# lemma-osu/sknnr

Hardware: AMD Instinct MI355X
Metric: Mqueries/sec + achieved HBM GB/s, 10M×50k×32 k=5, 1/2/4/8 MI355X (higher is better)
Workload: dtype f16 split MFMA (hi.hi swept, lo.hi + hi.lo corrections; f32 accumulate) pre-filter + f64 exact re-score

## Files before the change

include/sknnr_hip.h:

```cpp
#ifndef SKNNR_HIP_H
#define SKNNR_HIP_H

#include <stdint.h>

#ifdef __cplusplus
extern "C" {
#endif
#pragma GCC visibility push(default)

#define SKNNR_ABI_VERSION 5

typedef enum sknnr_status {
    SKNNR_OK = 0,
    SKNNR_ERR_INVALID = -1,
    SKNNR_ERR_K_TOO_LARGE = -2,
    SKNNR_ERR_NO_TARGETS = -3,
    SKNNR_ERR_UNSUPPORTED = -4,
    SKNNR_ERR_HIP = -5,
    SKNNR_ERR_NO_DEVICE = -6,
    SKNNR_ERR_NONFINITE = -7
} sknnr_status;

typedef enum sknnr_memspace {
    SKNNR_MEM_HOST = 0,
// ... 124 lines not shown
int sknnr_crosswalk(const int64_t* table, int64_t n_table, const int64_t* idx, int64_t n,
                    int64_t* out, int32_t device, int32_t mem, void* stream);


int sknnr_debug_coarse_matrix(sknnr_index* index, const double* q, int64_t nq, float* out,
                              double* out_qnorm, double* out_scale, double* out_eps);

int sknnr_debug_last_prefilter(const sknnr_index* index, int64_t out[8]);

int sknnr_debug_last_finalize(const sknnr_index* index, int64_t out[4]);

int sknnr_debug_last_hamming(const sknnr_index* index, int64_t out[8]);

int sknnr_debug_last_scan(const sknnr_index* index, int64_t out[8]);

int sknnr_debug_hamming_candidates(const sknnr_index* index, int32_t* cnt, int32_t* ids, int64_t n);

int sknnr_debug_last_prep(const sknnr_index* index, int64_t out[8]);

int sknnr_debug_query_prep(const sknnr_index* index, int64_t n, void* qimg, double* qnc, double* xt, uint8_t* cell,
                           int32_t* perm, double* qnc_pos);

int sknnr_debug_image_constants(const sknnr_index* index, double* mu, double* s, int32_t* cell_depth, float* axes,
                                float* centre, float* thr);

#pragma GCC visibility pop
#ifdef __cplusplus
}
#endif
#endif
// ... 1 lines not shown
```

sknnr_amd/_build.py:

```python

from __future__ import annotations

import hashlib
import os
import shutil
import subprocess
import sys
from concurrent.futures import ThreadPoolExecutor

CSRC = os.path.join(os.path.dirname(os.path.abspath(__file__)), "csrc")
LIB_NAME = "libsknnr_hip.so"
LIB_PATH = os.path.join(CSRC, LIB_NAME)
OBJ_DIR = os.path.join(CSRC, "_obj")
UNITS = [
    ("host", "sknnr_hip.hip", []),
    ("k_exact", "k_exact.hip", []),
    ("k_hamming", "k_hamming.hip", []),
    ("k_forest", "k_forest.hip", []),
    ("k_coarse1", "k_coarse1.hip", []),
    ("k_coarse2_a", "k_coarse2.hip", ["-DSKNNR_C2_PART=0"]),
    ("k_coarse2_b", "k_coarse2.hip", ["-DSKNNR_C2_PART=1"]),
]
SOURCES = sorted({u[1] for u in UNITS})
HEADERS = ["launch.hip.h", "coarse.hip.h", "coarse2.hip.h", "bucket.hip.h", "hamming.hip.h", "exact.hip.h", "forest.hip.h",
           "../../include/sknnr_hip.h"]

HIPCC_FLAGS = [
    "--offload-arch=gfx950",
    "-O3",
    "-std=c++17",
    "-fPIC",
    "-ffp-contract=off",
    "-fvisibility=hidden",
    "-Wall",
    "-Wno-unused-function",
]


def hipcc_path() -> str:
# ... 71 lines not shown
```

sknnr_amd/_native.py:

```python

from __future__ import annotations

import ctypes
import os
from ctypes import POINTER, byref, c_char_p, c_double, c_float, c_int32, c_int64, c_void_p

import numpy as np

from . import _build

MEM_HOST = 0
MEM_DEVICE = 1
FORMULA_EXPANDED = 0
FORMULA_DIRECT = 1
FORMULA_HAMMING = 2
WEIGHTS_UNIFORM = 0
WEIGHTS_DISTANCE = 1
WEIGHTS_EXPLICIT = 2
WEIGHTS_F32_TARGETS = 0x100
WEIGHTS_F32_WEIGHTS = 0x200

ERR_INVALID = -1
ERR_K_TOO_LARGE = -2
ERR_NO_TARGETS = -3
# ... 37 lines not shown
    "sknnr_predict",
    "sknnr_predict_from_neighbors",
    "sknnr_hamming_distances",
    "sknnr_shard_candidates",
    "sknnr_merge_shards",
    "sknnr_stream_begin",
    "sknnr_stream_push",
    "sknnr_stream_flush",
    "sknnr_stream_end",
    "sknnr_crosswalk",
    "sknnr_debug_coarse_matrix",
    "sknnr_debug_last_prefilter",
    "sknnr_debug_last_finalize",
    "sknnr_debug_last_hamming",
    "sknnr_debug_last_scan",
    "sknnr_debug_hamming_candidates",
    "sknnr_debug_last_prep",
    "sknnr_debug_query_prep",
    "sknnr_debug_image_constants",
)


class QueryOpts(ctypes.Structure):
    _fields_ = [
        ("n_neighbors", c_int32),
        ("exclude_self", c_int32),
        ("deterministic", c_int32),
        ("decimals", c_int32),
        ("formula", c_int32),
        ("apply_affine", c_int32),
# ... 84 lines not shown
    lib.sknnr_predict.argtypes = [vp, vp, c_int64, POINTER(QueryOpts), vp, vp, vp, c_int32, vp]
    lib.sknnr_predict_from_neighbors.argtypes = [vp, vp, vp, vp, c_int64, c_int32, c_int32, vp,
                                                 c_int32, vp]
    lib.sknnr_hamming_distances.argtypes = [vp, vp, c_int64, vp, c_int64, vp, c_int32, vp]
    lib.sknnr_shard_candidates.argtypes = [vp, vp, c_int64, POINTER(QueryOpts), c_int64, vp, vp, c_int32, vp]
    lib.sknnr_merge_shards.argtypes = [vp, vp, c_int64, POINTER(QueryOpts), c_int32, vp, vp, vp, vp, c_int32, vp]
    lib.sknnr_crosswalk.argtypes = [vp, c_int64, vp, c_int64, vp, c_int32, c_int32, vp]
    lib.sknnr_debug_coarse_matrix.argtypes = [vp, vp, c_int64, vp, vp, POINTER(c_double),
                                              POINTER(c_double)]
    lib.sknnr_debug_last_prefilter.argtypes = [vp, POINTER(c_int64)]
    if hasattr(lib, "sknnr_debug_last_finalize"):
        lib.sknnr_debug_last_finalize.argtypes = [vp, POINTER(c_int64)]
    lib.sknnr_debug_last_hamming.argtypes = [vp, POINTER(c_int64)]
    if hasattr(lib, "sknnr_debug_last_scan"):
        lib.sknnr_debug_last_scan.argtypes = [vp, POINTER(c_int64)]
    lib.sknnr_debug_hamming_candidates.argtypes = [vp, vp, vp, c_int64]
    if hasattr(lib, "sknnr_debug_last_prep"):
        lib.sknnr_debug_last_prep.argtypes = [vp, POINTER(c_int64)]
        lib.sknnr_debug_query_prep.argtypes = [vp, c_int64, vp, vp, vp, vp, vp, vp]
        lib.sknnr_debug_image_constants.argtypes = [vp, vp, POINTER(c_double), POINTER(c_int32), vp, vp, vp]
    _lib = lib
    return lib


def check(code: int) -> None:
    if code != 0:
        raise HipBackendError(code, load().sknnr_last_error().decode("utf-8", "replace"))


def device_count() -> int:
# ... 81 lines not shown

    def forest_apply_host(self, q, query_dtype=0):
        q = _c_rows(q, QueryOpts(query_dtype=int(query_dtype)))
        out = np.empty((q.shape[0], self.d), dtype=np.float64)
        check(load().sknnr_forest_apply(self.handle, _host_ptr(q), q.shape[0], int(query_dtype), MEM_HOST,
                                        _host_ptr(out)))
        return out

    def forest_apply_device(self, q_ptr, nq, query_dtype, out_ptr):
        check(load().sknnr_forest_apply(self.handle, c_void_p(q_ptr or None), nq, int(query_dtype), MEM_DEVICE,
                                        c_void_p(out_ptr or None)))

    def stats(self) -> dict:
        st = Stats()
        check(load().sknnr_get_stats(self.handle, byref(st)))
        return st.as_dict()

    def reset_stats(self):
        check(load().sknnr_reset_stats(self.handle))

    @staticmethod
    def make_opts(k, exclude_self=False, deterministic=True, decimals=10, formula=FORMULA_EXPANDED,
                  apply_affine=False, weight_mode=WEIGHTS_UNIFORM, row_offset=0,
                  check_finite=False, query_dtype=0) -> QueryOpts:
        return QueryOpts(int(k), int(bool(exclude_self)), int(bool(deterministic)), int(decimals),
                         int(formula), int(bool(apply_affine)), int(weight_mode), int(bool(check_finite)),
                         int(query_dtype), 0, int(row_offset))

    def check_finite(self, stream=0) -> None:
        check(load().sknnr_check_finite(self.handle, c_void_p(stream or None)))

# ... 118 lines not shown
        return dict(zip(self.FINALIZE_FIELDS, (int(v) for v in out)))

    HAMMING_FIELDS = ("ran", "kk", "compacts", "seed_rows", "band", "tree_pairs", "chunks", "handed_to_scan")

    def debug_last_hamming(self) -> dict:
        out = (c_int64 * 8)()
        check(load().sknnr_debug_last_hamming(self.handle, out))
        return dict(zip(self.HAMMING_FIELDS, (int(v) for v in out)))

    SCAN_FIELDS = ("formula_plus_1", "chunked", "kk", "workgroups", "lds_bytes", "rows", "slices", "replayed_rows")

    def debug_last_scan(self) -> dict:
        out = (c_int64 * 8)()
        check(load().sknnr_debug_last_scan(self.handle, out))
        return dict(zip(self.SCAN_FIELDS, (int(v) for v in out)))

    def debug_hamming_candidates(self, n: int):
        cnt = np.empty(n, dtype=np.int32)
        ids = np.empty((n, 192), dtype=np.int32)
        check(load().sknnr_debug_hamming_candidates(self.handle, _host_ptr(cnt), _host_ptr(ids), int(n)))
        return cnt, ids

    PREP_FIELDS = ("kernel", "rows_per_block", "x_dtype", "nq", "nq_pad", "xt_written", "cells_by", "affine_bits")

    def debug_last_prep(self) -> dict:
        out = (c_int64 * 8)()
        check(load().sknnr_debug_last_prep(self.handle, out))
        return dict(zip(self.PREP_FIELDS, (int(v) for v in out)))

    def debug_query_prep(self, n: int, want=("qimg", "qnc", "xt", "cell", "perm", "qnc_pos")) -> dict:
# ... 124 lines not shown
```

sknnr_amd/csrc/exact.hip.h:

```cpp
#pragma once
#include <type_traits>
#include <hip/hip_runtime.h>
#include <float.h>
#include <math.h>
#include <stdint.h>

#include "bucket.hip.h"
#include "coarse.hip.h"

namespace sknnr {

enum : int { kDtypeF64 = 0, kDtypeF32 = 1, kDtypeI16 = 2, kDtypeU16 = 3, kDtypeU8 = 4, kDtypeI32 = 5, kDtypeCount = 6 };
__host__ __device__ constexpr int dtype_bytes(int dt) {
    return dt == kDtypeF64 ? 8 : (dt == kDtypeF32 || dt == kDtypeI32 ? 4 : (dt == kDtypeU8 ? 1 : 2));
}
__device__ __forceinline__ double load_as_f64(const void* __restrict__ x, int dt, long i) {
    switch (dt) {
        case kDtypeF32: return (double)((const float*)x)[i];
        case kDtypeI16: return (double)((const short*)x)[i];
        case kDtypeU16: return (double)((const unsigned short*)x)[i];
        case kDtypeU8: return (double)((const unsigned char*)x)[i];
        case kDtypeI32: return (double)((const int*)x)[i];
        default: return ((const double*)x)[i];
    }
// ... 356 lines not shown
    double s2;
    double inv_s;
    double eps_c;
    double ymax;
    double noise_a;
    double mu2;
    int* fail_list;
    int fail_base;
    int* fail_count;
    const int* qperm;
    long pos0;
    const unsigned long long* rec;
    const float* rec_bound;
    const double* qnc_pos;
    int* trunc_count;
};

constexpr int kDppQuadXor[4] = {0xE4, 0xB1, 0x4E, 0x1B};
constexpr int kDppRowHalfMirror = 0x141;
__device__ __forceinline__ int half_mirror8(int v) { return __builtin_amdgcn_update_dpp(0, v, kDppRowHalfMirror, 0xf, 0xf, false); }
template <int N>
__device__ __forceinline__ int peer8_i(int v, int mirror) {
    static_assert(N >= 1 && N < 8, "a peer of an 8-lane group");
    if constexpr (N < 4) {
        return __builtin_amdgcn_update_dpp(0, v, kDppQuadXor[N], 0xf, 0xf, false);
    } else if constexpr (N < 7) {
        return __builtin_amdgcn_update_dpp(0, mirror, kDppQuadXor[7 - N], 0xf, 0xf, false);
    } else {
        return mirror;
    }
}
// ... 202 lines not shown
    const double tau = group_min<LPQ>(rank >= s.kk - 1 ? d2 : INFINITY, c);
    const double bound = (qn + t_min - eps) * a.inv_s2 - noise;
    bool certified = (n_usable >= s.kk) && (tau < INFINITY) && (bound > tau);
    bool truncated = false;
    if constexpr (RECORD) {
        truncated = group_any<LPQ>(c == LPQ - 1 && need, (int)(threadIdx.x & 63) & ~(LPQ - 1));
        if (truncated) certified = false;
    }
    {
        const int gbase = (int)(threadIdx.x & 63) & ~(LPQ - 1);
        const double by_rank = scatter_d<LPQ>(d2, gbase + rank);
        const double next = __shfl_down(by_rank, 1, LPQ);
        const bool has_next = c + 1 < LPQ;
        const bool tied_here = has_next && by_rank == next && by_rank < INFINITY &&
                               (s.deterministic ? c == s.kk - 1 : c < s.kk);
        if (!s.raw && group_any<LPQ>(tied_here, gbase)) certified = false;
    }

    int sel = rank;
    const long self_id = s.row_offset + q;
    if (s.exclude_self) {
        const bool is_self = usable && (long)id == self_id && rank < s.kk;
        int drop = group_min_i<LPQ>(is_self ? rank : 0x7fffffff, c);
        if (drop == 0x7fffffff) drop = 0;
        sel = rank == drop ? -1 : (rank > drop ? rank - 1 : rank);
    }
    const bool chosen = usable && sel >= 0 && sel < s.k;
    const double dist = s.raw ? d2 : sqrt(d2 > 0.0 ? d2 : 0.0);

    int pos = sel;
    if (s.deterministic) {
// ... 13 lines not shown
            const PeersL<LPQ> k1_of(k1);
            const PeersI<LPQ> tag_of(tagged);
            for_each_peer<LPQ>([&](auto n) {
                const double k0j = k0_of.template get<n.value>();
                const long k1j = k1_of.template get<n.value>();
                const int tj = tag_of.template get<n.value>();
                const int ij = tj & 0x7fffffff;
                const bool less = (k0j < k0) || (k0j == k0 && (k1j < k1 || (k1j == k1 && ij < key_id)));
                pos += (tj < 0) && less;
            });
        }
    }
    if (live && chosen) {
        if (s.out_dist) s.out_dist[q * s.k + pos] = dist;
        s.out_idx[q * s.k + pos] = id + s.id_offset;
    }
    if (live && c == 0 && !certified) {
        const int slot = atomicAdd(a.fail_count, 1);
        a.fail_list[slot] = a.fail_base + (int)q;
        if (RECORD && truncated) atomicAdd(a.trunc_count, 1);
    }
}

#ifdef SKNNR_KERNELS_EXACT
__global__ void __launch_bounds__(256) finalize_record_kernel(FinalizeArgs a) {
    constexpr int LPQ = kRecordLen;
    const SelectArgs& s = a.s;
    const long gt = (long)blockIdx.x * 256 + threadIdx.x;
    long q = gt / LPQ;
    const int c = (int)(gt % LPQ);
    const bool live = q < s.nq;
    if (!live) q = s.nq - 1;
    const long q_list = a.qperm ? a.pos0 + q : q;
    const unsigned long long e = a.rec[q_list * LPQ + c];
    const float t_min = a.rec_bound[q_list];
// ... 684 lines not shown
```

sknnr_amd/csrc/k_exact.hip:

```cpp
#define SKNNR_KERNELS_EXACT 1
#include <cstdint>
#include <cstdlib>

#include "launch.hip.h"

namespace sknnr {
namespace {
__global__ void add_counter_kernel(const int* __restrict__ cnt, long long* __restrict__ total) { *total += *cnt; }

template <int BT>
hipError_t prep_lds_bt(const PrepArgs& a, hipStream_t st) {
    const size_t sh = (size_t)BT * (a.d_in | 1) * 8;
    hipError_t e = hipFuncSetAttribute((const void*)prep_queries_kernel<BT>, hipFuncAttributeMaxDynamicSharedMemorySize, (int)sh);
    if (e != hipSuccess) return e;
    prep_queries_kernel<BT><<<dim3((unsigned)(a.nq_pad / BT)), dim3(BT), sh, st>>>(a);
    return hipGetLastError();
}

template <int FORMULA>
hipError_t exact_scan_f(bool chunked, const ScanArgs& a, long blocks, size_t sh, hipStream_t st) {
    auto kern = chunked ? exact_scan_kernel<FORMULA, true> : exact_scan_kernel<FORMULA, false>;
    hipError_t e = hipFuncSetAttribute((const void*)kern, hipFuncAttributeMaxDynamicSharedMemorySize, (int)sh);
    if (e != hipSuccess) return e;
    kern<<<dim3((unsigned)blocks), dim3(kScanWaves * 64), sh, st>>>(a);
// ... 109 lines not shown
    return hipGetLastError();
}

hipError_t crosswalk(const long* table, const long* idx, long n, long* out, hipStream_t st) {
    const long want = (n + 255) / 256;
    const unsigned blocks = (unsigned)(want < 1 ? 1 : (want > 256L * 16 ? 256L * 16 : want));
    crosswalk_kernel<<<dim3(blocks), dim3(256), 0, st>>>(table, idx, n, out);
    return hipGetLastError();
}

hipError_t add_counter(const int* cnt, long long* total, hipStream_t st) {
    add_counter_kernel<<<dim3(1), dim3(1), 0, st>>>(cnt, total);
    return hipGetLastError();
}

}
}
```

sknnr_amd/csrc/launch.hip.h:

```cpp
#pragma once
#include <hip/hip_runtime.h>

#include "bucket.hip.h"
#include "coarse2.hip.h"
#include "exact.hip.h"
#include "forest.hip.h"
#include "hamming.hip.h"

namespace sknnr {
namespace launch {

hipError_t row_norms(const double* x, long n, int d, double* out, hipStream_t st);
hipError_t prep_direct(const PrepArgs& a, hipStream_t st);
hipError_t prep_lds(int rows_per_block, const PrepArgs& a, hipStream_t st);
hipError_t check_finite(const double* x, long n_el, int* status, hipStream_t st);
hipError_t cell_assign(const CellArgs& a, hipStream_t st);
hipError_t cell_count(const CellArgs& a, hipStream_t st);
hipError_t cell_scatter(const CellArgs& a, hipStream_t st);
hipError_t finalize(const FinalizeArgs& f, long n, hipStream_t st);
int finalize_lanes(const FinalizeArgs& f);
hipError_t exact_scan(int formula, bool chunked, const ScanArgs& a, long blocks, size_t lds_bytes, hipStream_t st);
hipError_t scan_merge(int formula, const ScanArgs& a, long blocks, size_t lds_bytes, int grid_wg_of_scan, int forced_slices,
                      hipStream_t st);
hipError_t pack_shards(const double* val, const long* idx, long nq, int n_shards, int kk, double* slice_v, int* slice_i,
                       hipStream_t st);
hipError_t predict(const PredictArgs& a, hipStream_t st);
hipError_t crosswalk(const long* table, const long* idx, long n, long* out, hipStream_t st);
hipError_t add_counter(const int* cnt, long long* total, hipStream_t st);

hipError_t hamming_pack(const double* xq, long nq, long nq_pad, int t, int tp, uint32_t* qimg, int* q_bad, hipStream_t st);
hipError_t hamming_rows(const double* x, long n, int t, int tpr, uint32_t* rows, hipStream_t st);
hipError_t hamming_coarse(const HammingArgs& a, hipStream_t st);
hipError_t hamming_rescore(const HammingRescoreArgs& a, hipStream_t st);
hipError_t hamming_distance_rows(const HammingRowsArgs& a, hipStream_t st);

hipError_t forest_apply(const ForestArgs& a, hipStream_t st);

struct Coarse1Launch {
    const char* rimg;
    int n_stages;
    const uint4* qimg;
    const double* qnc;
    float skip_scale;
// ... 33 lines not shown
```

sknnr_amd/csrc/sknnr_hip.hip:

```cpp
#include "../../include/sknnr_hip.h"

#include <hip/hip_runtime.h>
#include <sys/mman.h>

#include <algorithm>
#include <chrono>
#include <cmath>
#include <cstdarg>
#include <cstdio>
#include <cstdlib>
#include <condition_variable>
#include <cstring>
#include <deque>
#include <functional>
#include <future>
#include <limits>
#include <memory>
#include <mutex>
#include <new>
#include <string>
#include <thread>
#include <vector>

#include "launch.hip.h"
// ... 190 lines not shown
    DevBuf<int> perm2;
    int cell_depth = 0;
    DevBuf<float> cell_axes, cell_centre, cell_thr;
    DevBuf<int> cell_stage;
    DevBuf<unsigned char> qcell;
    DevBuf<int> qperm, cell_hist;

    DevBuf<double> xt, qnc, xstage, dist_stage, pred_stage;
    DevBuf<uint4> qimg;
    DevBuf<float> cand_val;
    DevBuf<int> cand_idx, fail_list, fail_count, fail_list2, slice_i;
    DevBuf<unsigned long long> rec;
    DevBuf<float> rec_bound;
    DevBuf<double> qnc_pos;
    DevBuf<double> slice_v;
    DevBuf<int> status;
    DevBuf<long long> fail_total;
    DevBuf<long> idx_stage;

    struct HostSlot {
        double* pin_x = nullptr;  size_t pin_x_n = 0;
        double* pin_d = nullptr;  size_t pin_d_n = 0;
        long* pin_i = nullptr;    size_t pin_i_n = 0;
        double* pin_p = nullptr;  size_t pin_p_n = 0;
        DevBuf<double> dev_x, dev_d, dev_p;
        DevBuf<long> dev_i;
        hipEvent_t ev_h2d = nullptr, ev_done = nullptr, ev_d2h = nullptr;
    } slot[kHostSlots];
    hipStream_t st_h2d = nullptr, st_run = nullptr, st_d2h = nullptr;
    std::unique_ptr<HostWorker> w_in, w_out;
// ... 34 lines not shown
                        &dist_stage, &pred_stage, &f_ids})
            b->release();
        f_nodes.release(); f_off.release(); f_depth.release();
        rimg.release();
        perm.release();
        perm2.release();
        cell_axes.release(); cell_centre.release(); cell_thr.release(); cell_stage.release();
        qcell.release(); qperm.release(); cell_hist.release();
        h_rimg.release(); h_wq.release(); h_qimg.release(); h_rrow.release(); h_bad.release(); h_cand_cnt.release(); h_cand_id.release();
        qimg.release();
        cand_val.release();
        cand_idx.release();
        rec.release(); rec_bound.release(); qnc_pos.release();
        fail_list.release();
        fail_count.release();
        fail_total.release();
        status.release();
        idx_stage.release();
        for (auto& sl : slot) {
            for (void* hp : {(void*)sl.pin_x, (void*)sl.pin_d, (void*)sl.pin_i, (void*)sl.pin_p})
                if (hp) (void)hipHostFree(hp);
            sl.dev_x.release(); sl.dev_d.release(); sl.dev_p.release(); sl.dev_i.release();
            for (hipEvent_t e : {sl.ev_h2d, sl.ev_done, sl.ev_d2h})
                if (e) (void)hipEventDestroy(e);
        }
        for (hipStream_t h : {st_h2d, st_run, st_d2h})
            if (h) (void)hipStreamDestroy(h);
        if (ev_ws) (void)hipEventDestroy(ev_ws);
        if (st_side) (void)hipStreamDestroy(st_side);
        for (hipEvent_t e : {ev_fork, ev_join})
// ... 507 lines not shown
        }
        {
            double m2 = 0.0;
            for (int c = 0; c < d; ++c) m2 += ix->mu[c] * ix->mu[c];
            ix->mu_norm = std::sqrt(m2) * (1.0 + 1e-12);
        }
        HIP_TRY(ix->rimg.ensure(img.size()));
        HIP_TRY(hipMemcpy(ix->rimg.p, img.data(), img.size(), hipMemcpyHostToDevice));
        HIP_TRY(ix->perm.ensure((size_t)n_ref));
        HIP_TRY(hipMemcpy(ix->perm.p, perm.data(), (size_t)n_ref * sizeof(int), hipMemcpyHostToDevice));
        HIP_TRY(ix->mu_dev.ensure(dp));
        HIP_TRY(hipMemcpy(ix->mu_dev.p, ix->mu.data(), dp * sizeof(double), hipMemcpyHostToDevice));
    }

    HIP_TRY(ix->fail_count.ensure(4));
    HIP_TRY(ix->fail_total.ensure(2));
    HIP_TRY(hipMemset(ix->fail_total.p, 0, 16));
    HIP_TRY(ix->status.ensure(4));
    HIP_TRY(hipMemset(ix->status.p, 0, 16));
    HIP_TRY(hipEventCreateWithFlags(&ix->ev_ws, hipEventDisableTiming));
    HIP_TRY(hipDeviceSynchronize());
    guard.p = nullptr;
    *out = ix;
    return SKNNR_OK;
}

extern "C" void sknnr_index_destroy(sknnr_index* ix) { delete ix; }

extern "C" int sknnr_index_set_affine(sknnr_index* ix, int32_t d_in, const double* center,
                                      const double* scale, const double* proj) {
// ... 546 lines not shown
        return fail(SKNNR_ERR_UNSUPPORTED, "n_neighbors = %d exceeds the HIP backend's limit of %d%s", o->n_neighbors,
                    kScanMaxKK - (o->exclude_self ? 1 : 0),
                    o->exclude_self ? " with X=None (the query rows' own rows are searched too)" : "");
    if (std::abs(o->decimals) > 300) return fail(SKNNR_ERR_INVALID, "decimals out of range");
    return SKNNR_OK;
}

int run_forest(sknnr_index* ix, const void* xdev, long nq, const sknnr_query_opts* o, double* d_dist, long* d_idx,
               hipStream_t st);
int run_device(sknnr_index* ix, const void* xdev, long nq, const sknnr_query_opts* o, double* d_dist,
               long* d_idx, hipStream_t st, int raw = 0, long id_offset = 0) {
    std::fill(std::begin(ix->last_prefilter), std::end(ix->last_prefilter), 0);
    std::fill(std::begin(ix->last_hamming), std::end(ix->last_hamming), 0);
    std::fill(std::begin(ix->last_finalize), std::end(ix->last_finalize), 0);
    std::fill(std::begin(ix->last_scan), std::end(ix->last_scan), 0);
    std::fill(std::begin(ix->last_prep), std::end(ix->last_prep), 0);
    ix->last_hamming_rows = 0;
    if (xdev && uses_forest(ix, o)) return run_forest(ix, xdev, nq, o, d_dist, d_idx, st);
    const int kk = o->n_neighbors + (o->exclude_self ? 1 : 0);
    const bool affine = o->apply_affine != 0 && xdev != nullptr;
    const bool self_rows = xdev == nullptr;
    const int x_dtype = self_rows ? kDtypeF64 : o->query_dtype;
    const bool to_xt = affine || x_dtype != kDtypeF64;
    static const bool scan_everything = std::getenv("SKNNR_EXACT_ONLY") != nullptr;
    const bool coarse = ix->ks > 0 && kk <= kCoarseMaxKK && o->formula != SKNNR_FORMULA_HAMMING && !scan_everything;
    const int d_x = affine ? ix->d_in : ix->d;
    if (nq > 0x7fffffffL) return fail(SKNNR_ERR_UNSUPPORTED, "more than 2^31 - 1 query rows in one call");
    if (affine && ix->ks == 0)
        return fail(SKNNR_ERR_UNSUPPORTED, "d = %d > 128 with an affine map is outside the HIP envelope", ix->d);
    if (ix->ws_busy) HIP_TRY(hipStreamWaitEvent(st, ix->ev_ws, 0));
// ... 15 lines not shown
        HIP_TRY(ix->qcell.ensure((size_t)cap_pad));
        HIP_TRY(ix->qperm.ensure((size_t)cap_pad));
    }
    const bool record = coarse && use_record(ix->ks, coarse_list_len(ix, kk), kk, use_coarse2(ix, coarse_list_len(ix, kk)), raw);
    if (record) {
        HIP_TRY(ix->rec.ensure((size_t)cap_pad * kRecordLen));
        HIP_TRY(ix->rec_bound.ensure((size_t)cap_pad));
        if (ix->cell_depth > 0) HIP_TRY(ix->qnc_pos.ensure((size_t)cap_pad));
    } else if (coarse) {
        HIP_TRY(ix->cand_val.ensure((size_t)cap_pad * 2 * coarse_list_len(ix, kk)));
        HIP_TRY(ix->cand_idx.ensure((size_t)cap_pad * 2 * coarse_list_len(ix, kk)));
    }
    if (coarse) {
        HIP_TRY(ix->fail_list.ensure(nq));
        HIP_TRY(hipMemsetAsync(ix->fail_count.p, 0, 16, st));
    }

    SelectArgs call{};
    call.xq = xq_call;
    call.ref = ix->ref64.p;
    call.rn = ix->rn64.p;
    call.nq = nq;
    call.d = ix->d;
    call.n_ref = (int)ix->n_ref;
    call.k = o->n_neighbors;
    call.kk = kk;
    call.exclude_self = o->exclude_self ? 1 : 0;
    call.deterministic = o->deterministic ? 1 : 0;
    call.formula = o->formula;
    call.pow10_is_divisor = o->decimals < 0;
// ... 106 lines not shown
            f.rec_bound = ix->rec_bound.p;
            f.qnc_pos = bucketed ? ix->qnc_pos.p : ix->qnc.p;
            f.trunc_count = ix->fail_count.p + 3;
        }
        f.m_list = coarse_list_len(ix, kk);
        f.rank_extra = coarse_rank_extra(f.m_list, kk);
        f.inv_s2 = 1.0 / (ix->s * ix->s);
        f.s2 = ix->s * ix->s;
        f.inv_s = 1.0 / ix->s;
        f.eps_c = (v2 ? eps_units2(ix->ks) : eps_units(ix->ks)) * std::ldexp(1.0, -24);
        f.ymax = ix->ymax;
        f.noise_a = (ix->d + 4) * std::ldexp(1.0, -53);
        f.mu2 = o->formula == SKNNR_FORMULA_EXPANDED ? 2.0 * ix->mu_norm : 0.0;
        f.fail_list = ix->fail_list.p;
        f.fail_count = ix->fail_count.p;
        f.fail_base = (int)c0;
        auto finalize_rows = [&](long r0, long rows, hipStream_t s_) {
            FinalizeArgs g = f;
            if (bucketed) {
                g.pos0 = r0;
                g.s.nq = rows;
                launch_finalize(g, rows, s_);
                return;
            }
            g.s.xq = f.s.xq + r0 * ix->d;
            g.s.nq = rows;
            g.s.row_offset = f.s.row_offset + r0;
            g.s.out_dist = f.s.out_dist ? f.s.out_dist + r0 * o->n_neighbors : nullptr;
            g.s.out_idx = f.s.out_idx + r0 * o->n_neighbors;
            if (record) {
// ... 10 lines not shown
        };
        ix->last_finalize[0] = launch::finalize_lanes(f);
        ix->last_finalize[1] = record ? 1 : 0;
        const long done = v2 ? std::min<long>(ix->bulk_rows_done, n) : 0;
        if (done > 0) {
            HIP_TRY(hipStreamWaitEvent(ix->st_side, ix->ev_fork, 0));
            finalize_rows(0, done, ix->st_side);
            HIP_TRY(hipGetLastError());
            HIP_TRY(hipEventRecord(ix->ev_join, ix->st_side));
            if (n > done) finalize_rows(done, n - done, st);
            HIP_TRY(hipGetLastError());
            HIP_TRY(hipStreamWaitEvent(st, ix->ev_join, 0));
        } else {
            finalize_rows(0, n, st);
            HIP_TRY(hipGetLastError());
        }
    }
    const bool ham_int = !coarse && o->formula == SKNNR_FORMULA_HAMMING && ix->h16_ok && kk <= kHamMaxKK;
    if (ham_int) {
        const long chunk_q = 1L << 18;
        const long cap_q = std::min(chunk_q, nq);
        const long cap_pad = (cap_q + 255) / 256 * 256;
        HIP_TRY(ix->h_qimg.ensure((size_t)ix->h_tp * cap_pad));
        HIP_TRY(ix->h_bad.ensure((size_t)cap_pad));
        HIP_TRY(ix->h_cand_cnt.ensure((size_t)cap_q));
        HIP_TRY(ix->h_cand_id.ensure((size_t)cap_q * kHamCand));
        HIP_TRY(ix->fail_list.ensure(nq));
        HIP_TRY(hipMemsetAsync(ix->fail_count.p, 0, 16, st));
        const int64_t rec[7] = {1, kk, ham_compacts(kk) ? 1 : 0, ham_seed_rows((int)ix->n_ref, kk), (int64_t)ix->d + 2,
                                ix->h_tp, (nq + chunk_q - 1) / chunk_q};
// ... 23 lines not shown
            hr.s.xq = xq_call + c0 * ix->d;
            hr.s.nq = n;
            hr.s.row_offset = o->row_offset + c0;
            hr.s.out_dist = d_dist ? d_dist + c0 * o->n_neighbors : nullptr;
            hr.s.out_idx = d_idx + c0 * o->n_neighbors;
            hr.cand_cnt = ix->h_cand_cnt.p;
            hr.cand_id = ix->h_cand_id.p;
            hr.fail_list = ix->fail_list.p;
            hr.fail_count = ix->fail_count.p;
            hr.fail_base = (int)c0;
            hr.rrow = ix->h_rrow.p;
            hr.tpr = ham_row_dwords(ix->d);
            HIP_TRY(launch::hamming_rescore(hr, st));
        }
    }
    int rc = (coarse || ham_int) ? launch_scan(ix, call, ix->fail_list.p, ix->fail_count.p, nq, st)
                                 : launch_scan(ix, call, nullptr, nullptr, nq, st);
    if (rc) return rc;
    if (coarse) {
        HIP_TRY(launch::add_counter(ix->fail_count.p, ix->fail_total.p, st));
        ix->stats.coarse_queries += nq;
    } else {
        if (ham_int) HIP_TRY(launch::add_counter(ix->fail_count.p, ix->fail_total.p, st));
        ix->stats.exact_only_queries += nq;
    }
    HIP_TRY(hipEventRecord(ct.e1, st));
    ct.pending = true;
    HIP_TRY(hipEventRecord(ix->ev_ws, st));
    ix->ws_busy = true;
    ix->stats.queries += nq;
    return SKNNR_OK;
}

long forest_chunk_rows(int n_trees) {
    const long by_bytes = (4L << 30) / (8L * std::max(n_trees, 1));
// ... 572 lines not shown
    if (sh > 150 * 1024) return fail(SKNNR_ERR_UNSUPPORTED, "n_neighbors = %d with d = %d does not fit the exact scan kernel", call.k, call.d);
    ScanArgs b{call, ix->refT.p, ix->fail_list2.p, ix->fail_count.p + 2, nullptr, nullptr, nullptr, nullptr};
    const bool chunked = call.d > kScanColChunk;
    const int nq_pass = scan_nq(call.formula);
    const long blocks = std::max<long>(1, std::min<long>((nq + nq_pass - 1) / nq_pass, kScanGridWg));
    const int64_t rec[8] = {call.formula + 1, chunked ? 1 : 0, call.kk, blocks, (int64_t)sh, nq, n_shards, 1};
    std::copy(std::begin(rec), std::end(rec), ix->last_scan);
    HIP_TRY(launch::exact_scan(call.formula, chunked, b, blocks, sh, st));
    return SKNNR_OK;
}

int merge_shards_device(sknnr_index* ix, const double* xdev, long nq, const sknnr_query_opts* o, int n_shards,
                        const double* shard_val, const long* shard_idx, double* d_dist, long* d_idx, hipStream_t st) {
    std::fill(std::begin(ix->last_prefilter), std::end(ix->last_prefilter), 0);
    std::fill(std::begin(ix->last_scan), std::end(ix->last_scan), 0);
    std::fill(std::begin(ix->last_prep), std::end(ix->last_prep), 0);
    const int kk = o->n_neighbors + (o->exclude_self ? 1 : 0);
    const bool affine = o->apply_affine != 0 && xdev != nullptr;
    const bool self_rows = xdev == nullptr;
    if (nq > 0x7fffffffL) return fail(SKNNR_ERR_UNSUPPORTED, "more than 2^31 - 1 query rows in one call");
    if (affine && ix->ks == 0) return fail(SKNNR_ERR_UNSUPPORTED, "d = %d > 128 with an affine map is outside the HIP envelope", ix->d);
    if (ix->ws_busy) HIP_TRY(hipStreamWaitEvent(st, ix->ev_ws, 0));
    const double* xq_call = self_rows ? ix->ref64.p + o->row_offset * ix->d : xdev;
    if (affine) {
        HIP_TRY(ix->xt.ensure((size_t)nq * ix->d));
        const long chunk = chunk_rows(ix->ks, 2);
        const long cap_pad = (std::min(chunk, nq) + kRowQuantum - 1) / kRowQuantum * kRowQuantum;
        HIP_TRY(ix->qimg.ensure((size_t)(cap_pad / 32) * 2 * ix->ks * 64));
        HIP_TRY(ix->qnc.ensure(cap_pad));
        for (long c0 = 0; c0 < nq; c0 += chunk) {
// ... 361 lines not shown

extern "C" int sknnr_debug_last_scan(const sknnr_index* cix, int64_t out[8]) {
    if (!cix || !out) return fail(SKNNR_ERR_INVALID, "NULL argument");
    sknnr_index* ix = const_cast<sknnr_index*>(cix);
    std::lock_guard<std::mutex> lock(ix->mtx);
    const int64_t* r = ix->last_scan;
    std::copy(r, r + 8, out);
    out[7] = 0;
    if (!r[0]) return SKNNR_OK;
    if (r[5] < 0 || r[7]) {
        int cnt[3] = {0, 0, 0};
        HIP_TRY(hipSetDevice(ix->device));
        HIP_TRY(hipDeviceSynchronize());
        HIP_TRY(hipMemcpy(cnt, ix->fail_count.p, sizeof cnt, hipMemcpyDeviceToHost));
        if (r[5] < 0) out[5] = cnt[0];
        if (r[7]) out[7] = cnt[2];
    }
    if (!r[6]) out[6] = scan_slices(out[5], scan_nq((int)r[0] - 1), (int)ix->n_ref, (int)r[2], (int)r[3]);
    return SKNNR_OK;
}

extern "C" int sknnr_debug_hamming_candidates(const sknnr_index* cix, int32_t* cnt, int32_t* ids, int64_t n) {
    if (!cix || !cnt || !ids) return fail(SKNNR_ERR_INVALID, "NULL argument");
    sknnr_index* ix = const_cast<sknnr_index*>(cix);
    std::lock_guard<std::mutex> lock(ix->mtx);
    if (!ix->last_hamming[0]) return fail(SKNNR_ERR_INVALID, "the last call did not run the integer Hamming pre-filter");
    if (n < 0 || n > ix->last_hamming_rows)
        return fail(SKNNR_ERR_INVALID, "n = %ld rows, the last device chunk has %ld", (long)n, ix->last_hamming_rows);
    HIP_TRY(hipSetDevice(ix->device));
    HIP_TRY(hipDeviceSynchronize());
    HIP_TRY(hipMemcpy(cnt, ix->h_cand_cnt.p, (size_t)n * sizeof(int32_t), hipMemcpyDeviceToHost));
    HIP_TRY(hipMemcpy(ids, ix->h_cand_id.p, (size_t)n * kHamCand * sizeof(int32_t), hipMemcpyDeviceToHost));
    return SKNNR_OK;
// ... 51 lines not shown
```

Baseline: 221.3.

## Add MFMA rescue pass to resolve coarse-filter failures before exact scan

Queries the coarse pre-filter cannot certify now get a per-query float threshold computed in finalize. A new rescue kernel re-sweeps the f16 reference tiles with MFMA for those failed queries only, collecting up to 16 candidates under the threshold and re-finalizing them exactly. Only rows that still fail are handed to the expensive exact f64 scan. This adds an extra full-tile sweep kernel per chunk, plus atomics and state bookkeeping, in exchange for shrinking the exact-scan fallback list. It is on by default and can be disabled with the SKNNR_RESCUE environment variable.

```diff
diff --git a/include/sknnr_hip.h b/include/sknnr_hip.h
--- a/include/sknnr_hip.h
+++ b/include/sknnr_hip.h
@@ -162,6 +162,8 @@
 
 int sknnr_debug_last_scan(const sknnr_index* index, int64_t out[8]);
 
+int sknnr_debug_last_rescue(const sknnr_index* index, int64_t out[8]);
+
 int sknnr_debug_hamming_candidates(const sknnr_index* index, int32_t* cnt, int32_t* ids, int64_t n);
 
 int sknnr_debug_last_prep(const sknnr_index* index, int64_t out[8]);
diff --git a/sknnr_amd/_build.py b/sknnr_amd/_build.py
--- a/sknnr_amd/_build.py
+++ b/sknnr_amd/_build.py
@@ -22,7 +22,7 @@
     ("k_coarse2_b", "k_coarse2.hip", ["-DSKNNR_C2_PART=1"]),
 ]
 SOURCES = sorted({u[1] for u in UNITS})
-HEADERS = ["launch.hip.h", "coarse.hip.h", "coarse2.hip.h", "bucket.hip.h", "hamming.hip.h", "exact.hip.h", "forest.hip.h",
+HEADERS = ["launch.hip.h", "coarse.hip.h", "coarse2.hip.h", "bucket.hip.h", "hamming.hip.h", "exact.hip.h", "rescue.hip.h", "forest.hip.h",
            "../../include/sknnr_hip.h"]
 
 HIPCC_FLAGS = [
diff --git a/sknnr_amd/_native.py b/sknnr_amd/_native.py
--- a/sknnr_amd/_native.py
+++ b/sknnr_amd/_native.py
@@ -75,6 +75,7 @@
     "sknnr_debug_last_finalize",
     "sknnr_debug_last_hamming",
     "sknnr_debug_last_scan",
+    "sknnr_debug_last_rescue",
     "sknnr_debug_hamming_candidates",
     "sknnr_debug_last_prep",
     "sknnr_debug_query_prep",
@@ -189,6 +190,8 @@
     lib.sknnr_debug_last_hamming.argtypes = [vp, POINTER(c_int64)]
     if hasattr(lib, "sknnr_debug_last_scan"):
         lib.sknnr_debug_last_scan.argtypes = [vp, POINTER(c_int64)]
+    if hasattr(lib, "sknnr_debug_last_rescue"):
+        lib.sknnr_debug_last_rescue.argtypes = [vp, POINTER(c_int64)]
     lib.sknnr_debug_hamming_candidates.argtypes = [vp, vp, vp, c_int64]
     if hasattr(lib, "sknnr_debug_last_prep"):
         lib.sknnr_debug_last_prep.argtypes = [vp, POINTER(c_int64)]
@@ -300,7 +303,10 @@
     def stats(self) -> dict:
         st = Stats()
         check(load().sknnr_get_stats(self.handle, byref(st)))
-        return st.as_dict()
+        out = st.as_dict()
+        if hasattr(load(), "sknnr_debug_last_rescue"):
+            out["rescued_rows"] = self.debug_last_rescue()["rescued_total"]
+        return out
 
     def reset_stats(self):
         check(load().sknnr_reset_stats(self.handle))
@@ -449,6 +455,13 @@
         out = (c_int64 * 8)()
         check(load().sknnr_debug_last_scan(self.handle, out))
         return dict(zip(self.SCAN_FIELDS, (int(v) for v in out)))
+
+    RESCUE_FIELDS = ("launched", "ks", "offered", "not_rescuable", "overflowed", "rescued", "handed_on", "rescued_total")
+
+    def debug_last_rescue(self) -> dict:
+        out = (c_int64 * 8)()
+        check(load().sknnr_debug_last_rescue(self.handle, out))
+        return dict(zip(self.RESCUE_FIELDS, (int(v) for v in out)))
 
     def debug_hamming_candidates(self, n: int):
         cnt = np.empty(n, dtype=np.int32)
diff --git a/sknnr_amd/csrc/exact.hip.h b/sknnr_amd/csrc/exact.hip.h
--- a/sknnr_amd/csrc/exact.hip.h
+++ b/sknnr_amd/csrc/exact.hip.h
@@ -394,7 +394,17 @@
     const float* rec_bound;
     const double* qnc_pos;
     int* trunc_count;
+    float* fail_thr;
 };
+
+__device__ __forceinline__ float rescue_threshold(double qn, double tau, double eps, double noise, double s2, double inv_s2) {
+    const double t0 = ((tau + noise) * s2 + eps) - qn;
+    float t = (float)t0;
+    if (!((double)t > t0)) t = nextafterf(t, INFINITY);
+    t = nextafterf(t, INFINITY);
+    const bool ok = (qn + (double)t - eps) * inv_s2 - noise > tau;
+    return ok && t < INFINITY && qn < INFINITY && tau < INFINITY ? t : __builtin_nanf("");
+}
 
 constexpr int kDppQuadXor[4] = {0xE4, 0xB1, 0x4E, 0x1B};
 constexpr int kDppRowHalfMirror = 0x141;
@@ -627,7 +637,17 @@
         const bool has_next = c + 1 < LPQ;
         const bool tied_here = has_next && by_rank == next && by_rank < INFINITY &&
                                (s.deterministic ? c == s.kk - 1 : c < s.kk);
-        if (!s.raw && group_any<LPQ>(tied_here, gbase)) certified = false;
+        const bool tied = group_any<LPQ>(tied_here, gbase);
+        if (!s.raw && tied) certified = false;
+        if (live && c == 0 && !certified) {
+            const int slot = atomicAdd(a.fail_count, 1);
+            a.fail_list[slot] = a.fail_base + (int)q;
+            if (a.fail_thr) {
+                const bool rescuable = n_usable >= s.kk && tau < INFINITY && qn < INFINITY && !tied;
+                a.fail_thr[slot] = rescuable ? rescue_threshold(qn, tau, eps, noise, a.s2, a.inv_s2) : __builtin_nanf("");
+            }
+            if (RECORD && truncated) atomicAdd(a.trunc_count, 1);
+        }
     }
 
     int sel = rank;
@@ -671,11 +691,6 @@
     if (live && chosen) {
         if (s.out_dist) s.out_dist[q * s.k + pos] = dist;
         s.out_idx[q * s.k + pos] = id + s.id_offset;
-    }
-    if (live && c == 0 && !certified) {
-        const int slot = atomicAdd(a.fail_count, 1);
-        a.fail_list[slot] = a.fail_base + (int)q;
-        if (RECORD && truncated) atomicAdd(a.trunc_count, 1);
     }
 }
 
diff --git a/sknnr_amd/csrc/k_exact.hip b/sknnr_amd/csrc/k_exact.hip
--- a/sknnr_amd/csrc/k_exact.hip
+++ b/sknnr_amd/csrc/k_exact.hip
@@ -147,5 +147,26 @@
     return hipGetLastError();
 }
 
+template <int KS>
+hipError_t rescue_ks(const RescueArgs& a, hipStream_t st) {
+    rescue_kernel<KS><<<dim3(kRescueGrid), dim3(kRescueWaves * 64), rescue_lds_bytes(a.f.s.d), st>>>(a);
+    return hipGetLastError();
+}
+
+hipError_t rescue(int ks, const RescueArgs& a, hipStream_t st) {
+    switch (ks) {
+        case 1: return rescue_ks<1>(a, st);
+        case 2: return rescue_ks<2>(a, st);
+        case 3: return rescue_ks<3>(a, st);
+        case 4: return rescue_ks<4>(a, st);
+    }
+    return hipErrorInvalidValue;
+}
+
+hipError_t rescue_account(const int* listed, const int* state, long long* total, hipStream_t st) {
+    rescue_account_kernel<<<dim3(1), dim3(1), 0, st>>>(listed, state, total);
+    return hipGetLastError();
+}
+
 }
 }
diff --git a/sknnr_amd/csrc/launch.hip.h b/sknnr_amd/csrc/launch.hip.h
--- a/sknnr_amd/csrc/launch.hip.h
+++ b/sknnr_amd/csrc/launch.hip.h
@@ -6,6 +6,7 @@
 #include "exact.hip.h"
 #include "forest.hip.h"
 #include "hamming.hip.h"
+#include "rescue.hip.h"
 
 namespace sknnr {
 namespace launch {
@@ -27,6 +28,8 @@
 hipError_t predict(const PredictArgs& a, hipStream_t st);
 hipError_t crosswalk(const long* table, const long* idx, long n, long* out, hipStream_t st);
 hipError_t add_counter(const int* cnt, long long* total, hipStream_t st);
+hipError_t rescue(int ks, const RescueArgs& a, hipStream_t st);
+hipError_t rescue_account(const int* listed, const int* state, long long* total, hipStream_t st);
 
 hipError_t hamming_pack(const double* xq, long nq, long nq_pad, int t, int tp, uint32_t* qimg, int* q_bad, hipStream_t st);
 hipError_t hamming_rows(const double* x, long n, int t, int tpr, uint32_t* rows, hipStream_t st);
diff --git a/sknnr_amd/csrc/rescue.hip.h b/sknnr_amd/csrc/rescue.hip.h
--- /dev/null
+++ b/sknnr_amd/csrc/rescue.hip.h
@@ -0,0 +1,168 @@
+#pragma once
+#include "coarse2.hip.h"
+#include "exact.hip.h"
+
+namespace sknnr {
+
+constexpr int kRescueCap = 16;
+constexpr int kRescueWaves = 8;
+constexpr int kRescueGrid = 512;
+constexpr int kRescueMaxKK = kRescueCap - 4;
+
+enum : int {
+    kRescueCursor = 0,
+    kRescueHanded = 1,
+    kRescueNoThr = 2,
+    kRescueOverflow = 3,
+    kRescueOffered = 4,
+    kRescueDone = 5,
+    kRescueWords = 8
+};
+
+struct RescueArgs {
+    FinalizeArgs f;
+    const char* rhi;
+    int n_tiles;
+    const int* perm;
+    const uint4* qimg;
+    const double* qnc;
+    int row0;
+    float skip_scale;
+    const int* list;
+    const float* thr;
+    const int* count;
+    int* state;
+};
+
+__host__ __device__ constexpr size_t rescue_lds_bytes(int d) { return 32 * 4 + 32 * kRescueCap * 4 + 32 * finalize_row_bytes(d); }
+
+template <int KS>
+__global__ void __launch_bounds__(kRescueWaves * 64, 4) rescue_kernel(RescueArgs a) {
+    constexpr int TB = tile2_bytes(KS);
+    constexpr int LPQ = kRescueCap;
+    static_assert(kRescueWaves * 64 == 32 * LPQ, "the finish gives every listed row of a block its group of lanes");
+    extern __shared__ __attribute__((aligned(16))) char resc_lds[];
+    int* cnt = (int*)resc_lds;
+    int* cand = cnt + 32;
+    char* xrows = (char*)(cand + 32 * kRescueCap);
+    const SelectArgs& s = a.f.s;
+    const int tid = threadIdx.x;
+    const int lane = tid & 63;
+    const int wave = __builtin_amdgcn_readfirstlane(tid >> 6);
+    const int half = lane >> 5, col = lane & 31;
+
+    const int begin = a.state[kRescueCursor], end = *a.count;
+    const int n_blocks = (end - begin + 31) / 32;
+    for (int blk = blockIdx.x; blk < n_blocks; blk += gridDim.x) {
+        const int item0 = begin + blk * 32;
+        __syncthreads();
+        if (tid < 32) cnt[tid] = 0;
+        __syncthreads();
+
+        {
+            const int item = item0 + col;
+            const bool on = item < end;
+            const float t = on ? a.thr[item] : __builtin_nanf("");
+            const bool swept = t == t;
+            const int r = swept ? a.list[item] - a.row0 : 0;
+            half8 bh[KS];
+#pragma unroll
+            for (int ks = 0; ks < KS; ++ks) bh[ks] = __builtin_bit_cast(half8, a.qimg[qimg_index(r, 0, KS, ks, half)]);
+            const float margin = a.skip_scale * (float)sqrt(a.qnc[r]) + 1e-30f;
+            float loose = swept ? t + margin : __builtin_nanf("");
+            auto unit = [&](int tile, const half8 (&ah)[KS], const floatx4 (&c0)[4]) {
+                floatx16 acc;
+#pragma unroll
+                for (int i = 0; i < 4; ++i) {
+                    acc[i] = c0[0][i];
+                    acc[4 + i] = c0[1][i];
+                    acc[8 + i] = c0[2][i];
+                    acc[12 + i] = c0[3][i];
+                }
+#pragma unroll
+                for (int ks = 0; ks < KS; ++ks) acc = __builtin_amdgcn_mfma_f32_32x32x16_f16(ah[ks], bh[ks], acc, 0, 0, 0);
+                bool any = false;
+#pragma unroll
+                for (int i = 0; i < 16; ++i) any |= acc[i] < loose;
+                if (__builtin_amdgcn_ballot_w64(any) == 0) return;
+#pragma unroll
+                for (int i = 0; i < 16; ++i) {
+                    if (acc[i] < loose) {
+                        const int pos = tile * 32 + acc_row(i, half);
+                        const int at = atomicAdd(&cnt[col], 1);
+                        if (at < kRescueCap) cand[col * kRescueCap + at] = pos < s.n_ref ? a.perm[pos] : -1;
+                        if (at >= kRescueCap) loose = __builtin_nanf("");
+                    }
+                }
+            };
+            auto load_tile = [&](int tile, half8 (&ah)[KS], floatx4 (&c0)[4]) {
+                const char* tb = a.rhi + (size_t)tile * TB;
+#pragma unroll
+                for (int ks = 0; ks < KS; ++ks) ah[ks] = *(const half8*)(tb + ks * 1024 + lane * 16);
+                const floatx4* cp = (const floatx4*)(tb + KS * 1024 + half * 64);
+#pragma unroll
+                for (int i = 0; i < 4; ++i) c0[i] = cp[i];
+            };
+            int tile = wave;
+            for (int trip = 0; tile < a.n_tiles; tile += 2 * kRescueWaves, ++trip) {
+                if ((trip & 7) == 0) {
+                    if (loose == loose && cnt[col] > kRescueCap) loose = __builtin_nanf("");
+                    if (__builtin_amdgcn_ballot_w64(loose == loose) == 0) break;
+                }
+                const int tile_b = tile + kRescueWaves;
+                half8 ah0[KS], ah1[KS];
+                floatx4 c00[4], c01[4];
+                load_tile(tile, ah0, c00);
+                if (tile_b < a.n_tiles) load_tile(tile_b, ah1, c01);
+                unit(tile, ah0, c00);
+                if (tile_b < a.n_tiles) unit(tile_b, ah1, c01);
+            }
+        }
+        __syncthreads();
+
+        {
+            const int qi = tid / LPQ, c = tid % LPQ;
+            const int item = item0 + qi;
+            const bool live = item < end;
+            const int it = live ? item : end - 1;
+            const long q = a.list[it];
+            const float t = a.thr[it];
+            const int n = cnt[qi];
+            double* xrow = (double*)(xrows + (size_t)qi * finalize_row_bytes(s.d));
+            for (int e = c; e < s.d; e += LPQ) xrow[e] = s.xq[q * s.d + e];
+            __builtin_amdgcn_fence(__ATOMIC_RELEASE, "wavefront");
+            __builtin_amdgcn_wave_barrier();
+            __builtin_amdgcn_fence(__ATOMIC_ACQUIRE, "wavefront");
+            const int id = c < (n < kRescueCap ? n : kRescueCap) ? cand[qi * kRescueCap + c] : -1;
+            const bool valid = id >= 0;
+            const bool overflowed = n > kRescueCap;
+            const unsigned long long head = __builtin_amdgcn_ballot_w64(live && c == 0);
+            const int n_nothr = __builtin_popcountll(__builtin_amdgcn_ballot_w64(live && c == 0 && !(t == t)));
+            const int n_over = __builtin_popcountll(__builtin_amdgcn_ballot_w64(live && c == 0 && overflowed));
+            if (lane == 0 && head != 0) {
+                if (n_nothr) atomicAdd(a.state + kRescueNoThr, n_nothr);
+                if (n_over) atomicAdd(a.state + kRescueOverflow, n_over);
+            }
+            finalize_core<LPQ, false>(a.f, q, c, live, xrow, id, valid, 0.f, a.qnc[q - a.row0], (double)INFINITY,
+                                      overflowed ? (double)__builtin_nanf("") : (double)t);
+        }
+    }
+    __syncthreads();
+    if (tid == 0) {
+        __threadfence();
+        if (atomicAdd(a.state + kRescueDone, 1) == (int)gridDim.x - 1) {
+            a.state[kRescueCursor] = end;
+            a.state[kRescueOffered] += end - begin;
+            a.state[kRescueDone] = 0;
+        }
+    }
+}
+
+#ifdef SKNNR_KERNELS_EXACT
+__global__ void rescue_account_kernel(const int* __restrict__ listed, const int* __restrict__ state, long long* __restrict__ total) {
+    total[0] += *listed;
+    total[1] += state[kRescueOffered] - state[kRescueHanded];
+}
+#endif
+
+}
diff --git a/sknnr_amd/csrc/sknnr_hip.hip b/sknnr_amd/csrc/sknnr_hip.hip
--- a/sknnr_amd/csrc/sknnr_hip.hip
+++ b/sknnr_amd/csrc/sknnr_hip.hip
@@ -228,6 +228,10 @@
     DevBuf<float> rec_bound;
     DevBuf<double> qnc_pos;
     DevBuf<double> slice_v;
+    DevBuf<float> fail_thr;
+    DevBuf<int> resc_list, resc_state;
+    bool rescue_enabled = true;
+    int64_t last_rescue[2] = {};
     DevBuf<int> status;
     DevBuf<long long> fail_total;
     DevBuf<long> idx_stage;
@@ -292,6 +296,7 @@
         rec.release(); rec_bound.release(); qnc_pos.release();
         fail_list.release();
         fail_count.release();
+        fail_thr.release(); resc_list.release(); resc_state.release();
         fail_total.release();
         status.release();
         idx_stage.release();
@@ -829,6 +834,11 @@
     }
 
     HIP_TRY(ix->fail_count.ensure(4));
+    HIP_TRY(ix->resc_state.ensure(kRescueWords));
+    {
+        const char* e = std::getenv("SKNNR_RESCUE");
+        ix->rescue_enabled = !(e && std::atoi(e) == 0);
+    }
     HIP_TRY(ix->fail_total.ensure(2));
     HIP_TRY(hipMemset(ix->fail_total.p, 0, 16));
     HIP_TRY(ix->status.ensure(4));
@@ -1405,6 +1415,7 @@
     std::fill(std::begin(ix->last_hamming), std::end(ix->last_hamming), 0);
     std::fill(std::begin(ix->last_finalize), std::end(ix->last_finalize), 0);
     std::fill(std::begin(ix->last_scan), std::end(ix->last_scan), 0);
+    std::fill(std::begin(ix->last_rescue), std::end(ix->last_rescue), 0);
     std::fill(std::begin(ix->last_prep), std::end(ix->last_prep), 0);
     ix->last_hamming_rows = 0;
     if (xdev && uses_forest(ix, o)) return run_forest(ix, xdev, nq, o, d_dist, d_idx, st);
@@ -1450,6 +1461,14 @@
     if (coarse) {
         HIP_TRY(ix->fail_list.ensure(nq));
         HIP_TRY(hipMemsetAsync(ix->fail_count.p, 0, 16, st));
+    }
+    const bool rescue = coarse && ix->rescue_enabled && !raw && kk <= kRescueMaxKK && use_coarse2(ix, coarse_list_len(ix, kk));
+    if (rescue) {
+        HIP_TRY(ix->fail_thr.ensure(nq));
+        HIP_TRY(ix->resc_list.ensure(nq));
+        HIP_TRY(hipMemsetAsync(ix->resc_state.p, 0, kRescueWords * sizeof(int), st));
+        ix->last_rescue[0] = 1;
+        ix->last_rescue[1] = ix->ks;
     }
 
     SelectArgs call{};
@@ -1586,6 +1605,7 @@
         f.mu2 = o->formula == SKNNR_FORMULA_EXPANDED ? 2.0 * ix->mu_norm : 0.0;
         f.fail_list = ix->fail_list.p;
         f.fail_count = ix->fail_count.p;
+        f.fail_thr = rescue ? ix->fail_thr.p : nullptr;
         f.fail_base = (int)c0;
         auto finalize_rows = [&](long r0, long rows, hipStream_t s_) {
             FinalizeArgs g = f;
@@ -1626,6 +1646,29 @@
         } else {
             finalize_rows(0, n, st);
             HIP_TRY(hipGetLastError());
+        }
+        if (rescue) {
+            RescueArgs ra{};
+            ra.f = f;
+            ra.f.s = call;
+            ra.f.fail_list = ix->resc_list.p;
+            ra.f.fail_count = ix->resc_state.p + kRescueHanded;
+            ra.f.fail_thr = nullptr;
+            ra.f.fail_base = 0;
+            ra.f.rec = nullptr;
+            ra.f.qperm = nullptr;
+            ra.rhi = ix->rhi2.p;
+            ra.n_tiles = ix->n_stages2 * tiles_per_stage2(ix->ks);
+            ra.perm = ix->perm2.p;
+            ra.qimg = ix->qimg.p;
+            ra.qnc = ix->qnc.p;
+            ra.row0 = (int)c0;
+            ra.skip_scale = (float)(std::ldexp(1.0, -9) * ix->ymax * 1.02);
+            ra.list = ix->fail_list.p;
+            ra.thr = ix->fail_thr.p;
+            ra.count = ix->fail_count.p;
+            ra.state = ix->resc_state.p;
+            HIP_TRY(launch::rescue(ix->ks, ra, st));
         }
     }
     const bool ham_int = !coarse && o->formula == SKNNR_FORMULA_HAMMING && ix->h16_ok && kk <= kHamMaxKK;
@@ -1679,11 +1722,13 @@
             HIP_TRY(launch::hamming_rescore(hr, st));
         }
     }
-    int rc = (coarse || ham_int) ? launch_scan(ix, call, ix->fail_list.p, ix->fail_count.p, nq, st)
-                                 : launch_scan(ix, call, nullptr, nullptr, nq, st);
+    int rc = rescue ? launch_scan(ix, call, ix->resc_list.p, ix->resc_state.p + kRescueHanded, nq, st)
+             : (coarse || ham_int) ? launch_scan(ix, call, ix->fail_list.p, ix->fail_count.p, nq, st)
+                                   : launch_scan(ix, call, nullptr, nullptr, nq, st);
     if (rc) return rc;
     if (coarse) {
-        HIP_TRY(launch::add_counter(ix->fail_count.p, ix->fail_total.p, st));
+        if (rescue) HIP_TRY(launch::rescue_account(ix->fail_count.p, ix->resc_state.p, ix->fail_total.p, st));
+        else HIP_TRY(launch::add_counter(ix->fail_count.p, ix->fail_total.p, st));
         ix->stats.coarse_queries += nq;
     } else {
         if (ham_int) HIP_TRY(launch::add_counter(ix->fail_count.p, ix->fail_total.p, st));
@@ -2286,6 +2331,7 @@
                         const double* shard_val, const long* shard_idx, double* d_dist, long* d_idx, hipStream_t st) {
     std::fill(std::begin(ix->last_prefilter), std::end(ix->last_prefilter), 0);
     std::fill(std::begin(ix->last_scan), std::end(ix->last_scan), 0);
+    std::fill(std::begin(ix->last_rescue), std::end(ix->last_rescue), 0);
     std::fill(std::begin(ix->last_prep), std::end(ix->last_prep), 0);
     const int kk = o->n_neighbors + (o->exclude_self ? 1 : 0);
     const bool affine = o->apply_affine != 0 && xdev != nullptr;
@@ -2677,9 +2723,37 @@
         HIP_TRY(hipDeviceSynchronize());
         HIP_TRY(hipMemcpy(cnt, ix->fail_count.p, sizeof cnt, hipMemcpyDeviceToHost));
         if (r[5] < 0) out[5] = cnt[0];
+        if (r[5] < 0 && ix->last_rescue[0]) {
+            int handed = 0;
+            HIP_TRY(hipMemcpy(&handed, ix->resc_state.p + kRescueHanded, sizeof handed, hipMemcpyDeviceToHost));
+            out[5] = handed;
+        }
         if (r[7]) out[7] = cnt[2];
     }
     if (!r[6]) out[6] = scan_slices(out[5], scan_nq((int)r[0] - 1), (int)ix->n_ref, (int)r[2], (int)r[3]);
+    return SKNNR_OK;
+}
+
+extern "C" int sknnr_debug_last_rescue(const sknnr_index* cix, int64_t out[8]) {
+    if (!cix || !out) return fail(SKNNR_ERR_INVALID, "NULL argument");
+    sknnr_index* ix = const_cast<sknnr_index*>(cix);
+    std::lock_guard<std::mutex> lock(ix->mtx);
+    std::fill(out, out + 8, 0);
+    HIP_TRY(hipSetDevice(ix->device));
+    HIP_TRY(hipDeviceSynchronize());
+    long long total[2] = {0, 0};
+    HIP_TRY(hipMemcpy(total, ix->fail_total.p, sizeof total, hipMemcpyDeviceToHost));
+    out[7] = total[1];
+    if (!ix->last_rescue[0]) return SKNNR_OK;
+    int w[kRescueWords];
+    HIP_TRY(hipMemcpy(w, ix->resc_state.p, sizeof w, hipMemcpyDeviceToHost));
+    out[0] = 1;
+    out[1] = ix->last_rescue[1];
+    out[2] = w[kRescueOffered];
+    out[3] = w[kRescueNoThr];
+    out[4] = w[kRescueOverflow];
+    out[5] = w[kRescueOffered] - w[kRescueHanded];
+    out[6] = w[kRescueHanded];
     return SKNNR_OK;
 }
 
```

New measurement: 226.0, median of 6. 1.02x the previous value.
